# cychomatica/AudioPure

Hardware: AMD Instinct MI355X
Metric: purified 1s@16kHz utterances/sec at 5 reverse steps (higher is better)
Workload: dtype f32

## Files before the change

__graft_entry__.py:

```python
from __future__ import annotations

import glob
import os
import subprocess
import sys

ROOT = os.path.dirname(os.path.abspath(__file__))
if ROOT not in sys.path:
    sys.path.insert(0, ROOT)

CSRC = os.path.join(ROOT, "audiopure_amd", "csrc")
LIBDIR = os.path.join(ROOT, "audiopure_amd", "lib")
LIB = os.path.join(LIBDIR, "libaudiopure_hip.so")
TOOLS_LIB = os.path.join(ROOT, "tools", "lib", "libaudiopure_hip_tools.so")
NO_SLP_VECTORIZE = {"ap_resblock_f32w.hip", "ap_resblock_bwd.hip", "ap_resblock_bwd_bf16.hip", "ap_conv_w3.hip", "ap_conv_p1.hip",
                    "ap_resblock_bf16p.hip", "ap_resblock_bf16s.hip", "ap_resblock_bf16u.hip", "ap_resblock_bf16us.hip",
                    "ap_resblock_bf16.hip", "ap_resblock_bf16w.hip", "ap_resblock_f32w_parent.hip"}
TOOLS_CSRC = os.path.join(ROOT, "tools", "csrc")
TOOLS_ONLY_SOURCES = ["ap_resblock_bf16.hip", "ap_resblock_bf16w.hip", "ap_skipgemm_bf16w.hip", "ap_conv_p1.hip",
                      "ap_resblock_f32w_parent.hip"]
HIP_SOURCES = ["ap_kernels.hip", "ap_resblock_f32w.hip", "ap_resblock_bwd.hip", "ap_resblock_bwd_bf16.hip", "ap_resblock_bf16p.hip", "ap_resblock_bf16s.hip", "ap_resblock_bf16u.hip", "ap_resblock_bf16us.hip", "ap_skipgemm_bf16.hip", "ap_resblock_f32s.hip", "ap_resblock_f32s2.hip", "ap_capi.hip", "ap_frontend.hip", "ap_mel.hip", "ap_convnet.hip", "ap_conv_w3.hip", "ap_backward.hip", "ap_kws.hip", "ap_unet_bwd.hip", "ap_defense.hip", "ap_psy.hip", "ap_wgrad.hip", "ap_m5_train.hip", "ap_convnet_train.hip", "ap_unet_train.hip", "ap_optim.hip", "ap_loss.hip"]


def _newer(target: str, sources) -> bool:
    if not os.path.exists(target):
        return False
    t = os.path.getmtime(target)
    return all(os.path.getmtime(s) <= t for s in sources)


def hip_flags(src: str, tools: bool = False) -> list:
    return (["--offload-arch=gfx950", "-O3", "-std=c++17", "-fPIC", "-I", CSRC] + (["-DAP_TOOLS"] if tools else [])
            + (["-fno-slp-vectorize"] if os.path.basename(src) in NO_SLP_VECTORIZE else []))


def build_hip(force: bool = False, tools: bool = False) -> str:
    lib = TOOLS_LIB if tools else LIB
    variant = os.environ.get("AP_VARIANT_LIB")
    if variant:
        lib, force = os.path.abspath(variant), True
    os.makedirs(os.path.dirname(lib), exist_ok=True)
    srcs = [os.path.join(CSRC, f) for f in HIP_SOURCES if os.path.exists(os.path.join(CSRC, f))]
    if tools:
        srcs += [os.path.join(TOOLS_CSRC, f) for f in TOOLS_ONLY_SOURCES]
    deps = srcs + glob.glob(os.path.join(CSRC, "*.h")) + [os.path.join(ROOT, "include", "audiopure.h")]
    if not force and _newer(lib, deps):
        return lib
    hipcc = os.environ.get("HIPCC", "/opt/rocm/bin/hipcc")
    objs = []
    procs = []
    for s in srcs:
        o = os.path.join(os.path.dirname(lib), os.path.basename(s) + (".tools.o" if tools else ".var.o" if variant else ".o"))
        objs.append(o)
        cmd = ([hipcc] + hip_flags(s, tools) + (os.environ.get("AP_VARIANT_FLAGS", "").split() if variant else []) + ["-c", s, "-o", o])
        procs.append((cmd, subprocess.Popen(cmd, stdout=subprocess.PIPE, stderr=subprocess.STDOUT)))
    for cmd, p in procs:
        out, _ = p.communicate()
        if p.returncode != 0:
            raise RuntimeError("hipcc failed: " + " ".join(cmd) + "\n" + out.decode(errors="replace"))
    cmd = [hipcc, "--offload-arch=gfx950", "-shared", "-fPIC", "-o", lib] + objs
    subprocess.run(cmd, check=True)
    for o in objs:
        os.remove(o)
    return lib


def build_oracle() -> None:
    mk = os.path.join(ROOT, "oracle", "Makefile")
    if os.path.exists(mk):
        subprocess.run(["make", "-s", "-C", os.path.join(ROOT, "oracle")], check=True)


def build() -> None:
    have_hipcc = os.path.exists(os.environ.get("HIPCC", "/opt/rocm/bin/hipcc"))
    build_hip(force=have_hipcc and os.environ.get("AP_BUILD_REUSE") != "1")
    build_oracle()
    import audiopure_amd
    from audiopure_amd import _native
    _native.lib()


def smoke() -> None:
    import numpy as np
    import torch

    from audiopure_amd import synth
    from audiopure_amd.diffusion_models.diffwave_ddpm import DiffWave
    from audiopure_amd.diffusion_models.DiffWave_Unconditional.WaveNet import WaveNet_Speech_Commands
    from audiopure_amd.diffusion_models.DiffWave_Unconditional.util import calc_diffusion_hyperparams
    from audiopure_amd.audio_models.M5.M5Net import M5
    from audiopure_amd.acoustic_system import AcousticSystem
    from oracle import diffwave_oracle as O

    assert torch.cuda.is_available(), "smoke() needs a GPU"
    dev = torch.device("cuda:0")
    cfg = synth.mini_wavenet_config(64, 12, 12)
    sd = synth.wavenet_state_dict(cfg, 0)
    net = WaveNet_Speech_Commands(**cfg)
    net.load_state_dict({k: torch.from_numpy(v) for k, v in sd.items()})
    net = net.to(dev)
    dh = calc_diffusion_hyperparams(**synth.DIFFUSION_CONFIG)
    B, L, n = 2, 16000, 2
    x0 = torch.from_numpy(synth.waveforms(B, L, seed=11))
    z = [torch.from_numpy(synth.noise(d, B, L, seed=11)) for d in range(n)]
    dw = DiffWave(model=net, diffusion_hyperparams=dh, reverse_timestep=n)
    dw.set_noise_source(list(t.to(dev) for t in z))
    m5sd = synth.m5_state_dict(10)
    m5 = M5(n_input=1, n_output=10)
    m5.load_state_dict({k: torch.from_numpy(np.asarray(v)) for k, v in m5sd.items()})
    m5 = m5.to(dev).eval()
    system = AcousticSystem(classifier=m5, transform=None, defender=dw, defense_type="wave")
    logp = system(x0.to(dev), True).cpu()
    x_ref, lp_ref = O.purify_and_classify(O.fold_state_dict(sd), cfg, O.diffusion_hyperparams(**synth.DIFFUSION_CONFIG),
                                          m5sd, x0, n, z)
    err = (logp - lp_ref).abs().max().item()
    assert err < 1e-3, f"smoke: log-prob mismatch {err}"
    print(f"smoke OK: max |dlogp| = {err:.2e}")


if __name__ == "__main__":
    if "--tools" in sys.argv:
        print("tools build OK:", build_hip(force=True, tools=True))
    else:
        build()
        print("build OK:", LIB)
```

audiopure_amd/csrc/ap_kernels.hip:

```cpp
#include "ap_common.h"

namespace ap {

__global__ void rownorm_kernel(const float *__restrict__ v, float *__restrict__ norm, int O, int IK) {
  int row = blockIdx.x * (blockDim.x >> 6) + (threadIdx.x >> 6);
  int lane = threadIdx.x & 63;
  if (row >= O) return;
  const float *p = v + (size_t)row * IK;
  float s = 0.f;
  for (int i = lane; i < IK; i += 64) s = __builtin_fmaf(p[i], p[i], s);
  for (int o = 32; o > 0; o >>= 1) s += __shfl_xor(s, o);
  if (lane == 0) norm[row] = sqrtf(s);
}

__global__ void fold_kernel(const float *__restrict__ g, const float *__restrict__ v,
                            const float *__restrict__ norm, float *__restrict__ out, int O, int IK) {
  size_t idx = (size_t)blockIdx.x * blockDim.x + threadIdx.x;
  if (idx >= (size_t)O * IK) return;
  int o = idx / IK;
  out[idx] = v[idx] * (g[o] / norm[o]);
}

__global__ void pack_w1_kernel(const float *__restrict__ w1f, float *__restrict__ out, int C) {
  const int NW = C / 64, NG = C * 3 / 8;
  size_t idx = (size_t)blockIdx.x * blockDim.x + threadIdx.x;
  size_t total = (size_t)NW * NG * 4 * 64 * 4;
  if (idx >= total) return;
  int e = idx & 3;
  int lane = (idx >> 2) & 63;
  int rt = (idx >> 8) & 3;
  size_t rest = idx >> 10;
  int G = rest % NG;
  int w = rest / NG;
  int s = 4 * G + e, hh = lane >> 5, i = lane & 31;
  int kk = 2 * s + hh;
  int chunk = kk / (3 * KC), within = kk % (3 * KC);
  int tap = within / KC, cl = within % KC;
  int c = chunk * KC + cl;
  int o = (rt & 1) * C + 64 * w + 32 * (rt >> 1) + i;
  out[idx] = w1f[((size_t)o * C + c) * 3 + tap];
}

__global__ void pack_rows_kernel(const float *__restrict__ wf, float *__restrict__ out, int M, int K, int RT,
                                 int mode) {
  const int NG = K / 8;
  const int NWv = M / (32 * RT);
  size_t idx = (size_t)blockIdx.x * blockDim.x + threadIdx.x;
  size_t total = (size_t)NWv * NG * RT * 64 * 4;
  if (idx >= total) return;
  int e = idx & 3;
  int lane = (idx >> 2) & 63;
  size_t rest = idx >> 8;
  int rt = rest % RT;
  rest /= RT;
  int G = rest % NG;
  int w = rest / NG;
  int s = 4 * G + e, hh = lane >> 5, i = lane & 31;
  int kk = 2 * s + hh;
  int o = 32 * RT * w + 32 * rt + i;
  if (mode == 1) o = (rt >> 1) * (M / 2) + 64 * w + 32 * (rt & 1) + i;
  out[idx] = wf[(size_t)o * K + kk];
}

__global__ void copy_kernel(const float *__restrict__ in, float *__restrict__ out, size_t n) {
  size_t idx = (size_t)blockIdx.x * blockDim.x + threadIdx.x;
  if (idx < n) out[idx] = in[idx];
}

static int fold_one(const float *g, const float *v, float *norms, float *out, int O, int IK, hipStream_t st) {
  rownorm_kernel<<<(O + 3) / 4, 256, 0, st>>>(v, norms, O, IK);
  size_t n = (size_t)O * IK;
  fold_kernel<<<(unsigned)((n + 255) / 256), 256, 0, st>>>(g, v, norms, out, O, IK);
  return 0;
}

static void copy_to(const float *in, float *out, size_t n, hipStream_t st) {
  copy_kernel<<<(unsigned)((n + 255) / 256), 256, 0, st>>>(in, out, n);
}

int launch_fold_and_pack(ap_ctx *ctx, const float *blob, hipStream_t st) {
  const ap_config &c = ctx->cfg;
  const int C = ctx->C, S = ctx->S, NL = ctx->NL;
  BlobLayout bl = blob_layout(c);
  fold_one(blob + bl.init_g, blob + bl.init_v, ctx->norms, ctx->w0, C, 1, st);
  copy_to(blob + bl.init_b, ctx->b0, C, st);
  copy_to(blob + bl.fc1_w, ctx->fc1_w, (size_t)c.embed_dim_mid * c.embed_dim_in, st);
  copy_to(blob + bl.fc1_b, ctx->fc1_b, c.embed_dim_mid, st);
  copy_to(blob + bl.fc2_w, ctx->fc2_w, (size_t)c.embed_dim_out * c.embed_dim_mid, st);
  copy_to(blob + bl.fc2_b, ctx->fc2_b, c.embed_dim_out, st);
  for (int n = 0; n < NL; n++) {
    const float *b = blob + bl.blk0 + (size_t)n * bl.blk_stride;
    copy_to(b + bl.fct_w, ctx->fct_w + (size_t)n * C * c.embed_dim_out, (size_t)C * c.embed_dim_out, st);
    copy_to(b + bl.fct_b, ctx->fct_b + (size_t)n * C, C, st);
    float *w1f = ctx->w1f + (size_t)n * 2 * C * C * 3;
    float *w2f = ctx->w2f + (size_t)n * (C + S) * C;
    fold_one(b + bl.dil_g, b + bl.dil_v, ctx->norms, w1f, 2 * C, C * 3, st);
    fold_one(b + bl.res_g, b + bl.res_v, ctx->norms, w2f, C, C, st);
    fold_one(b + bl.skip_g, b + bl.skip_v, ctx->norms, w2f + (size_t)C * C, S, C, st);
    copy_to(b + bl.dil_b, ctx->b1 + (size_t)n * 2 * C, 2 * C, st);
    copy_to(b + bl.res_b, ctx->b2 + (size_t)n * (C + S), C, st);
    copy_to(b + bl.skip_b, ctx->b2 + (size_t)n * (C + S) + C, S, st);
    size_t n1 = (size_t)2 * C * C * 3, n2 = (size_t)(C + S) * C;
    pack_w1_kernel<<<(unsigned)((n1 + 255) / 256), 256, 0, st>>>(w1f, ctx->w1p + (size_t)n * n1, C);
    pack_rows_kernel<<<(unsigned)((n2 + 255) / 256), 256, 0, st>>>(w2f, ctx->w2p + (size_t)n * n2, C + S, C, 4, 1);
  }
  fold_one(blob + bl.f1_g, blob + bl.f1_v, ctx->norms, ctx->wf1f, S, S, st);
  copy_to(blob + bl.f1_b, ctx->bf1, S, st);
  copy_to(blob + bl.f2_w, ctx->wf2, S, st);
  copy_to(blob + bl.f2_b, ctx->bf2, 1, st);
  size_t nf = (size_t)S * S;
  pack_rows_kernel<<<(unsigned)((nf + 255) / 256), 256, 0, st>>>(ctx->wf1f, ctx->wf1p, S, S, 2, 0);
  AP_HIP(hipGetLastError());
  return 0;
}

__device__ __forceinline__ float swish_acc(float x) { return x / (1.0f + expf(-x)); }

__global__ __launch_bounds__(512) void embed_mlp_kernel(const float *__restrict__ freq, const float *__restrict__ w1,
                                                        const float *__restrict__ b1, const float *__restrict__ w2,
                                                        const float *__restrict__ b2, float step, int Ein, int Emid,
                                                        int Eout, float *__restrict__ emb_out) {
  extern __shared__ float sm[];
  float *e0 = sm, *e1 = sm + Ein;
  const int lane = threadIdx.x & 63, wave = threadIdx.x >> 6;
  int half = Ein / 2;
  for (int i = threadIdx.x; i < half; i += blockDim.x) {
    float a = step * freq[i];
    e0[i] = sinf(a);
    e0[half + i] = cosf(a);
  }
  __syncthreads();
  for (int o0 = wave; o0 < Emid; o0 += 8 * 16) {
    float s[16];
#pragma unroll
    for (int i = 0; i < 16; i++) s[i] = 0.f;
    for (int kk = 0; kk < Ein; kk += 64) {
      const int k = min(kk + lane, Ein - 1);
      const float ev = kk + lane < Ein ? e0[k] : 0.f;
#pragma unroll
      for (int i = 0; i < 16; i++) s[i] = __builtin_fmaf(w1[(size_t)min(o0 + 8 * i, Emid - 1) * Ein + k], ev, s[i]);
    }
    for (int m = 32; m > 0; m >>= 1) {
#pragma unroll
      for (int i = 0; i < 16; i++) s[i] += __shfl_xor(s[i], m);
    }
    float mine = 0.f;
#pragma unroll
    for (int i = 0; i < 16; i++) mine = lane == i ? s[i] : mine;
    const int o = o0 + 8 * lane;
    if (lane < 16 && o < Emid) e1[o] = swish_acc(mine + b1[o]);
  }
  __syncthreads();
  const int o2 = min((int)blockIdx.x * 8 + wave, Eout - 1);
  float s = 0.f;
  for (int kk = 0; kk < Emid; kk += 512) {
    float wv[8];
#pragma unroll
    for (int i = 0; i < 8; i++) wv[i] = w2[(size_t)o2 * Emid + min(kk + 64 * i + lane, Emid - 1)];
#pragma unroll
    for (int i = 0; i < 8; i++) s = kk + 64 * i + lane < Emid ? __builtin_fmaf(wv[i], e1[kk + 64 * i + lane], s) : s;
  }
  for (int m = 32; m > 0; m >>= 1) s += __shfl_xor(s, m);
  if (lane == 0 && (int)blockIdx.x * 8 + wave < Eout) emb_out[o2] = swish_acc(s + b2[o2]);
}

__global__ void fct_kernel(const float *__restrict__ w, const float *__restrict__ b, const float *__restrict__ emb,
                           float *__restrict__ out, int rows, int E) {
  int row = blockIdx.x * (blockDim.x >> 6) + (threadIdx.x >> 6);
  int lane = threadIdx.x & 63;
  if (row >= rows) return;
  const float *p = w + (size_t)row * E;
  float s = 0.f;
  for (int i0 = 0; i0 < E; i0 += 512) {
    float wv[8], ev[8];
#pragma unroll
    for (int u = 0; u < 8; u++) {
      const int i = min(i0 + 64 * u + lane, E - 1);
      wv[u] = p[i];
      ev[u] = emb[i];
    }
#pragma unroll
    for (int u = 0; u < 8; u++) s = i0 + 64 * u + lane < E ? __builtin_fmaf(wv[u], ev[u], s) : s;
  }
  for (int o = 32; o > 0; o >>= 1) s += __shfl_xor(s, o);
  if (lane == 0) out[row] = s + b[row];
}

int launch_embed(ap_ctx *ctx, float step, float *part_t, hipStream_t st) {
  const ap_config &c = ctx->cfg;
  float *emb = part_t + (size_t)ctx->NL * ctx->C;
  size_t sm = (size_t)(c.embed_dim_in + c.embed_dim_mid) * sizeof(float);
  embed_mlp_kernel<<<(unsigned)((c.embed_dim_out + 7) / 8), 512, sm, st>>>(ctx->emb_freq, ctx->fc1_w, ctx->fc1_b, ctx->fc2_w, ctx->fc2_b, step,
                                       c.embed_dim_in, c.embed_dim_mid, c.embed_dim_out, emb);
  int rows = ctx->NL * ctx->C;
  fct_kernel<<<(rows + 3) / 4, 256, 0, st>>>(ctx->fct_w, ctx->fct_b, emb, part_t, rows, c.embed_dim_out);
  AP_HIP(hipGetLastError());
  return 0;
}

__global__ void init_conv_kernel(const float *__restrict__ x, const float *__restrict__ w0,
                                 const float *__restrict__ b0, float *__restrict__ h, int C, int L) {
  int b = blockIdx.z, c = blockIdx.y;
  int t = blockIdx.x * blockDim.x + threadIdx.x;
  if (t >= L) return;
  float v = __builtin_fmaf(w0[c], x[(size_t)b * L + t], b0[c]);
  h[((size_t)b * C + c) * L + t] = fmaxf(v, 0.f);
}

int launch_init_conv(ap_ctx *ctx, const float *x, float *h, int B, int L, hipStream_t st) {
  dim3 grid((L + 255) / 256, ctx->C, B);
  init_conv_kernel<<<grid, 256, 0, st>>>(x, ctx->w0, ctx->b0, h, ctx->C, L);
  AP_HIP(hipGetLastError());
  return 0;
}

template <int C, int TTK>
struct RBGeom {
  static constexpr int NWM = C / 64;
  static constexpr int NWN = TTK / 64;
  static constexpr int NW = NWM * NWN;
  static constexpr int NT = NW * 64;
  static constexpr int ROWS = 3 * KC;
  static constexpr int NCHUNK = C / KC;
  static constexpr int GPC = ROWS / 8;
  static constexpr int NG1 = NCHUNK * GPC;
  static constexpr int NG2 = C / 8;
  static constexpr int EPT = ROWS * TTK / NT;
  static constexpr int RPI = NT / TTK;
  static constexpr int NPT = KC / RPI;
  static constexpr int XBUF = ROWS * TTK;
  static constexpr int LDS_FLOATS = (2 * XBUF > C * TTK) ? 2 * XBUF : C * TTK;
};

template <int C, int TTK, bool SAVE = false>
__global__ __launch_bounds__(C / 64 * TTK, 2) void resblock_f32_kernel(
    const float *__restrict__ hin, const float *__restrict__ pt, float *__restrict__ hout, float *__restrict__ skip,
    const float *__restrict__ w1p, const float *__restrict__ b1, const float *__restrict__ w2p,
    const float *__restrict__ b2, int L, int d, int accumulate, int ntiles, float *__restrict__ aout AP_ABLATE_PARAM) {
  AP_ABLATE_DECL
  using G = RBGeom<C, TTK>;
  constexpr int TT = TTK;
  constexpr int NT = G::NT;
  __shared__ float lds[G::LDS_FLOATS];

  const int tid = threadIdx.x;
  const int lane = tid & 63;
  const int wave = __builtin_amdgcn_readfirstlane(tid >> 6);
  const int mw = wave / G::NWN, nw = wave % G::NWN;
  const int j = lane & 31, hh = lane >> 5;
  int b_, tile_;
  ap_tile_of_block(blockIdx.x, gridDim.x, ntiles, d, TT, b_, tile_);
  const int b = __builtin_amdgcn_readfirstlane(b_);
  const int t0 = __builtin_amdgcn_readfirstlane(tile_ * TT);
  const float *hin_b;
  {
    const uint64_t hb = (uint64_t)(hin + (size_t)b * C * L);
    const uint32_t lo = __builtin_amdgcn_readfirstlane((uint32_t)hb);
    const uint32_t hi = __builtin_amdgcn_readfirstlane((uint32_t)(hb >> 32));
    hin_b = (const float *)(((uint64_t)hi << 32) | lo);
  }

  f32x16 acc[4][2];
#pragma unroll
  for (int rt = 0; rt < 4; rt++) {
    const int obase = (rt & 1) * C + 64 * mw + 32 * (rt >> 1);
#pragma unroll
    for (int q = 0; q < 4; q++) {
      const float4 bv = *reinterpret_cast<const float4 *>(b1 + obase + 8 * q + 4 * hh);
#pragma unroll
      for (int ct = 0; ct < 2; ct++) {
        acc[rt][ct][4 * q + 0] = bv.x;
        acc[rt][ct][4 * q + 1] = bv.y;
        acc[rt][ct][4 * q + 2] = bv.z;
        acc[rt][ct][4 * q + 3] = bv.w;
      }
    }
  }

  constexpr int RPI = G::RPI, NPT = G::NPT;
  const int rsel = tid / TT;
  unsigned voff[3];
  bool tok[3];
#pragma unroll
  for (int tap = 0; tap < 3; tap++) {
    const int tp = t0 + (tid & (TT - 1)) + (tap - 1) * d;
    tok[tap] = (tp >= 0) && (tp < L);
    voff[tap] = ((unsigned)min(max(tp, 0), L - 1) + (unsigned)rsel * (unsigned)L) * 4u;
  }
  const __amdgpu_buffer_rsrc_t hrs =
      __builtin_amdgcn_make_buffer_rsrc((void *)hin_b, 0, (int)((unsigned)C * (unsigned)L * 4u), 0x00020000);
  float xr[G::EPT];
  float ptv[NPT];
  auto issue_loads = [&](int ch) {
#pragma unroll
    for (int q = 0; q < NPT; q++) ptv[q] = pt[ch * KC + q * RPI + rsel];
#pragma unroll
    for (int i = 0; i < G::EPT; i++) {
      const int rowc = i * RPI;
      const int tap = rowc / KC, clc = rowc % KC;
      const int soff = (ch * KC + clc) * L * 4;
      xr[i] = __builtin_bit_cast(float, __builtin_amdgcn_raw_buffer_load_b32(hrs, voff[tap], soff, 0));
    }
  };
  auto store_chunk = [&](float *dst) {
#pragma unroll
    for (int i = 0; i < G::EPT; i++) {
      const int rowc = i * RPI;
      const int tap = rowc / KC, clc = rowc % KC;
      const float u = xr[i] + ptv[clc / RPI];
      dst[i * NT + tid] = tok[tap] ? u : 0.f;
    }
  };

  issue_loads(0);
  store_chunk(lds);
  __syncthreads();

  auto load_a = [&](f32x4(&a)[4], const f32x4 *base, int Gi) {
#pragma unroll
    for (int rt = 0; rt < 4; rt++) a[rt] = base[(size_t)((ablate & 4) ? 0 : Gi) * 256 + rt * 64];
  };
  auto mma4 = [&](const f32x4(&a)[4], const float *xb) {
    float bv[4][2];
#pragma unroll
    for (int e = 0; e < 4; e++)
#pragma unroll
      for (int ct = 0; ct < 2; ct++) bv[e][ct] = xb[e * 2 * TT + 32 * ct];
#pragma unroll
    for (int e = 0; e < 4; e++)
#pragma unroll
      for (int rt = 0; rt < 4; rt++)
#pragma unroll
        for (int ct = 0; ct < 2; ct++)
          acc[rt][ct] = __builtin_amdgcn_mfma_f32_32x32x2f32(a[rt][e], bv[e][ct], acc[rt][ct], 0, 0, 0);
  };

  const int colbase = 64 * nw + j;
  const f32x4 *ap = reinterpret_cast<const f32x4 *>(w1p) + (size_t)mw * G::NG1 * 4 * 64 + lane;
  f32x4 a0[4], a1[4];
  load_a(a0, ap, 0);
  {
    static_assert(G::GPC % 2 == 0 && G::NG1 % 2 == 0, "pair-unrolled loop");
    int ch = 0, g = 0;
#pragma unroll 1
    for (int Gi = 0; Gi < G::NG1; Gi += 2) {
      load_a(a1, ap, Gi + 1);
      if (g == 0 && ch + 1 < G::NCHUNK && !(ablate & 8)) issue_loads(ch + 1);
      __builtin_amdgcn_sched_barrier(0);
      const float *xb = lds + (ch & 1) * G::XBUF + (g * 8 + hh) * TT + colbase;
      mma4(a0, xb);
      __builtin_amdgcn_sched_barrier(0);
      load_a(a0, ap, (Gi + 2 < G::NG1) ? Gi + 2 : Gi);
      __builtin_amdgcn_sched_barrier(0);
      mma4(a1, xb + 8 * TT);
      __builtin_amdgcn_sched_barrier(0);
      g += 2;
      if (g == G::GPC) {
        if (ch + 1 < G::NCHUNK) store_chunk(lds + ((ch + 1) & 1) * G::XBUF);
        __syncthreads();
        g = 0;
        ch++;
      }
    }
  }

#pragma unroll
  for (int p = 0; p < 2; p++)
#pragma unroll
    for (int ct = 0; ct < 2; ct++) {
#pragma unroll
      for (int r = 0; r < 16; r++) {
        const int c = 64 * mw + 32 * p + rowoff(r, hh);
        if constexpr (SAVE) {
          const int t = t0 + 32 * ct + colbase;
          if (t < L) {
            float *ab = aout + ((size_t)b * 2 * C + c) * L + t;
            ab[0] = acc[2 * p][ct][r];
            ab[(size_t)C * L] = acc[2 * p + 1][ct][r];
          }
        }
        lds[c * TT + 32 * ct + colbase] =
            (ablate & 2) ? acc[2 * p][ct][r] : gate(acc[2 * p][ct][r], acc[2 * p + 1][ct][r]);
      }
      __builtin_amdgcn_sched_barrier(0);
    }

  {
    const float *b2l = b2, *ptl = pt;
    asm volatile("" : "+s"(b2l), "+s"(ptl));
#pragma unroll
    for (int rt = 0; rt < 4; rt++) {
      const int cb = 64 * mw + 32 * (rt & 1);
#pragma unroll
      for (int q = 0; q < 4; q++) {
        const int c = cb + 8 * q + 4 * hh;
        float4 bv = *reinterpret_cast<const float4 *>(b2l + (rt < 2 ? 0 : C) + c);
        if (rt < 2) {
          const float4 pv = *reinterpret_cast<const float4 *>(ptl + c);
          bv.x += pv.x; bv.y += pv.y; bv.z += pv.z; bv.w += pv.w;
        }
#pragma unroll
        for (int ct = 0; ct < 2; ct++) {
          acc[rt][ct][4 * q + 0] = bv.x;
          acc[rt][ct][4 * q + 1] = bv.y;
          acc[rt][ct][4 * q + 2] = bv.z;
          acc[rt][ct][4 * q + 3] = bv.w;
        }
      }
    }
  }
  const f32x4 *ap2 = reinterpret_cast<const f32x4 *>(w2p) + (size_t)mw * G::NG2 * 4 * 64 + lane;
  load_a(a0, ap2, 0);
  load_a(a1, ap2, 1);
  __syncthreads();

  float hres[2][2][16];
  unsigned evoff[2][2];
#pragma unroll
  for (int rt = 0; rt < 2; rt++)
#pragma unroll
    for (int ct = 0; ct < 2; ct++) {
      const int t = min(t0 + 32 * ct + colbase, L - 1);
      evoff[rt][ct] = ((unsigned)(64 * mw + 32 * rt + 4 * hh) * (unsigned)L + (unsigned)t) * 4u;
    }
  if (!(ablate & 1)) {
#pragma unroll
    for (int rt = 0; rt < 2; rt++)
#pragma unroll
      for (int ct = 0; ct < 2; ct++)
#pragma unroll
        for (int r = 0; r < 16; r++)
          hres[rt][ct][r] = __builtin_bit_cast(
              float, __builtin_amdgcn_raw_buffer_load_b32(hrs, evoff[rt][ct], rowoff(r, 0) * L * 4, 2));
  }

  {
    static_assert(G::NG2 % 2 == 0, "pair-unrolled loop");
#pragma unroll 1
    for (int Gi = 0; Gi < G::NG2; Gi += 2) {
      const float *gb = lds + (Gi * 8 + hh) * TT + colbase;
      mma4(a0, gb);
      __builtin_amdgcn_sched_barrier(0);
      load_a(a0, ap2, (Gi + 2 < G::NG2) ? Gi + 2 : Gi);
      __builtin_amdgcn_sched_barrier(0);
      mma4(a1, gb + 8 * TT);
      __builtin_amdgcn_sched_barrier(0);
      load_a(a1, ap2, (Gi + 3 < G::NG2) ? Gi + 3 : Gi + 1);
      __builtin_amdgcn_sched_barrier(0);
    }
  }

  if (ablate & 1) return;
  const float RS = 0.707106781186547524f;
  float *ho = hout + (size_t)b * C * L;
  float *sk = skip + (size_t)b * C * L;
#pragma unroll
  for (int rt = 0; rt < 4; rt++) {
#pragma unroll
    for (int ct = 0; ct < 2; ct++) {
      const int t = t0 + 32 * ct + colbase;
      const unsigned rbase = (unsigned)(64 * mw + 32 * (rt & 1) + 4 * hh) * (unsigned)L + (unsigned)t;
      if (t < L) {
        if (rt < 2) {
#pragma unroll
          for (int r = 0; r < 16; r++)
            __builtin_nontemporal_store((hres[rt][ct][r] + acc[rt][ct][r]) * RS, &ho[rbase + (unsigned)rowoff(r, 0) * (unsigned)L]);
        } else if (accumulate) {
#pragma unroll
          for (int r = 0; r < 16; r++)
            unsafeAtomicAdd(&sk[rbase + (unsigned)rowoff(r, 0) * (unsigned)L], acc[rt][ct][r]);
        } else {
#pragma unroll
          for (int r = 0; r < 16; r++) __builtin_nontemporal_store(acc[rt][ct][r], &sk[rbase + (unsigned)rowoff(r, 0) * (unsigned)L]);
        }
      }
    }
  }
}

AP_TOOLS_VAR g_tile = 64;
AP_TOOLS_VAR g_force_direct = 0;
AP_TOOLS_VAR g_no_bf16s = 0;
AP_TOOLS_VAR g_force_f32 = 0;
#ifdef AP_TOOLS
static int g_ablate = 0;
#endif

int launch_resblock(ap_ctx *ctx, int layer, const float *hin, const float *pt, float *hout, float *skip,
                    int accumulate, int B, int L, hipStream_t st, float *aout, void *gout, void *fout) {
  if (aout && ctx->cfg.precision != AP_PREC_F32) {
    set_error("ap_resblock_fwd_save: AP_PREC_F32 only (the other modes recompute the pre-gate activations)");
    return -22;
  }
  if (ctx->cfg.precision == AP_PREC_BF16_STORE) {
    set_error("AP_PREC_BF16_STORE: the residual stream is a bf16 image in this mode (ap_init_conv_u / ap_resblock_fwd_u), not an fp32 tensor; "
              "the fp32-tensor block serves AP_PREC_F32, AP_PREC_F32_SPLIT and AP_PREC_BF16");
    return -22;
  }
  if (gout && (ctx->cfg.precision != AP_PREC_BF16 || g_force_f32)) {
    set_error("deferred-skip form: AP_PREC_BF16 only");
    return -22;
  }
  if (ctx->cfg.precision != AP_PREC_F32 && !g_force_f32) {
    ProfileSpan span;
    if (int e = span.begin(ctx, 0, st)) return e;
    int rc = ctx->cfg.precision == AP_PREC_BF16
                 ? (gout && !fout && g_no_bf16s != 1 && (g_no_bf16s == 2 || resblock_bf16s_serves(ctx, B, L))
                        ? launch_resblock_bf16s(ctx, layer, hin, pt, hout, gout, B, L, st)
                        : launch_resblock_bf16(ctx, layer, hin, pt, hout, skip, accumulate, B, L, st, gout, fout))
                 : launch_resblock_split(ctx, layer, hin, pt, hout, skip, accumulate, B, L, st);
    if (int e = span.end()) return e;
    return rc;
  }
  const int C = ctx->C, S = ctx->S;
  const int d = 1 << (layer % ctx->cfg.dilation_cycle);
  if (!g_force_direct && resblock_f32w_serves(ctx, B, L)) {
    ProfileSpan span;
    if (int e = span.begin(ctx, 0, st)) return e;
    const int rcw = launch_resblock_f32w(ctx, layer, hin, pt, hout, skip, accumulate, B, L, st, aout);
    if (int e = span.end()) return e;
    return rcw;
  }
  if (!hout) {
    set_error("resblock: the direct-form block needs an h' buffer");
    return -22;
  }
  const float *w1p = ctx->w1p + (size_t)layer * 2 * C * C * 3;
  const float *w2p = ctx->w2p + (size_t)layer * (C + S) * C;
  const float *b1 = ctx->b1 + (size_t)layer * 2 * C;
  const float *b2 = ctx->b2 + (size_t)layer * (C + S);
  ProfileSpan span;
  if (int e = span.begin(ctx, 0, st)) return e;
#define AP_RB(CC, TK)                                                                                              \
  resblock_f32_kernel<CC, TK><<<(unsigned)B * ((L + TK - 1) / TK), CC / 64 * TK, 0, st>>>(                         \
      hin, pt, hout, skip, w1p, b1, w2p, b2, L, d, accumulate, (L + TK - 1) / TK, nullptr AP_ABLATE_ARG(g_ablate))
#define AP_RB_SAVE(CC, TK)                                                                                         \
  resblock_f32_kernel<CC, TK, true><<<(unsigned)B * ((L + TK - 1) / TK), CC / 64 * TK, 0, st>>>(                   \
      hin, pt, hout, skip, w1p, b1, w2p, b2, L, d, accumulate, (L + TK - 1) / TK, aout AP_ABLATE_ARG(g_ablate))
  const int tk = g_tile;
  if (aout) {
    if (C == 256 && tk == 64) AP_RB_SAVE(256, 64);
    else if (C == 256) AP_RB_SAVE(256, 128);
    else if (C == 64) AP_RB_SAVE(64, 64);
    else {
      set_error("resblock (save): unsupported res_channels %d (need 64 or 256)", C);
      return -22;
    }
  } else
  if (C == 64 && tk == 64) AP_RB(64, 64);
  else if (C == 64) AP_RB(64, 128);
  else if (C == 128 && tk == 64) AP_RB(128, 64);
  else if (C == 128) AP_RB(128, 128);
  else if (C == 256 && tk == 64) AP_RB(256, 64);
  else if (C == 256) AP_RB(256, 128);
  else {
    set_error("resblock: unsupported res_channels %d (need 64, 128 or 256)", C);
    return -22;
  }
#undef AP_RB
#undef AP_RB_SAVE
  if (int e = span.end()) return e;
  AP_HIP(hipGetLastError());
  return 0;
}

__device__ __forceinline__ void philox4x32_10(uint32_t c0, uint32_t c1, uint32_t c2, uint32_t c3, uint32_t k0,
                                              uint32_t k1, uint32_t (&out)[4]) {
#pragma unroll
  for (int i = 0; i < 10; i++) {
    uint32_t hi0 = __umulhi(0xD2511F53u, c0), lo0 = 0xD2511F53u * c0;
    uint32_t hi1 = __umulhi(0xCD9E8D57u, c2), lo1 = 0xCD9E8D57u * c2;
    uint32_t n0 = hi1 ^ c1 ^ k0, n1 = lo1, n2 = hi0 ^ c3 ^ k1, n3 = lo0;
    c0 = n0; c1 = n1; c2 = n2; c3 = n3;
    k0 += 0x9E3779B9u;
    k1 += 0xBB67AE85u;
  }
  out[0] = c0; out[1] = c1; out[2] = c2; out[3] = c3;
}

__device__ __forceinline__ void philox_normal4(uint64_t seed, uint32_t draw, uint64_t utt, uint32_t quad,
                                               float (&z)[4]) {
  uint32_t r[4];
  philox4x32_10(quad, draw, (uint32_t)utt, (uint32_t)(utt >> 32), (uint32_t)seed, (uint32_t)(seed >> 32), r);
  const float TWO_PI = 6.283185307179586f;
#pragma unroll
  for (int p = 0; p < 2; p++) {
    float u1 = ((float)(r[2 * p] >> 9) + 0.5f) * 1.1920928955078125e-07f;
    float u2 = (float)(r[2 * p + 1] >> 8) * 5.9604644775390625e-08f;
    float rad = sqrtf(-2.0f * logf(u1));
    float sn, cs;
    sincosf(TWO_PI * u2, &sn, &cs);
    z[2 * p] = rad * cs;
    z[2 * p + 1] = rad * sn;
  }
}

__device__ __forceinline__ float philox_normal1(uint64_t seed, uint32_t draw, uint64_t utt, int t) {
  float z[4];
  philox_normal4(seed, draw, utt, (uint32_t)t >> 2, z);
  return z[t & 3];
}

__global__ void affine_noise_kernel(const float *__restrict__ x, float *__restrict__ out, float ca, float cs,
                                    const float *__restrict__ z, uint64_t seed, uint32_t draw, uint64_t utt_offset,
                                    int L) {
  const int b = blockIdx.y;
  const int q = blockIdx.x * blockDim.x + threadIdx.x;
  const int t = q * 4;
  if (t >= L) return;
  float zz[4];
  if (z == nullptr) {
    if (cs != 0.f) philox_normal4(seed, draw, utt_offset + b, (uint32_t)q, zz);
    else zz[0] = zz[1] = zz[2] = zz[3] = 0.f;
  }
#pragma unroll
  for (int i = 0; i < 4; i++) {
    if (t + i < L) {
      const size_t off = (size_t)b * L + t + i;
      float zv = z ? z[off] : zz[i];
      float xv = x ? x[off] : 0.f;
      out[off] = ca * xv + cs * zv;
    }
  }
}

int launch_affine_noise(const float *x, float *out, float ca, float cs, const float *z, uint64_t seed,
                        uint32_t draw, uint64_t utt_offset, int B, int L, hipStream_t st) {
  int quads = (L + 3) / 4;
  dim3 grid((quads + 255) / 256, B);
  affine_noise_kernel<<<grid, 256, 0, st>>>(x, out, ca, cs, z, seed, draw, utt_offset, L);
  AP_HIP(hipGetLastError());
  return 0;
}

template <int S, int FT>
__global__ __launch_bounds__(S / 64 * 64, FT == 64 ? 2 : 1) void final_f32_kernel(
    const float *__restrict__ skip, const float *__restrict__ x, float *__restrict__ eps_out, float *__restrict__ out,
    const float *__restrict__ wf1p, const float *__restrict__ bf1, const float *__restrict__ wf2,
    const float *__restrict__ bf2, float scale, float ca, float cb, float cs, const float *__restrict__ z,
    uint64_t seed, uint32_t draw, uint64_t utt_offset, int L, int ntiles) {
  constexpr int NW = S / 64, NT = NW * 64, NG = S / 8;
  constexpr int TT = FT, NCT = FT / 32;
  __shared__ float lds[S * TT];
  const int tid = threadIdx.x, lane = tid & 63;
  const int wave = __builtin_amdgcn_readfirstlane(tid >> 6);
  const int j = lane & 31, hh = lane >> 5;
  const int b = blockIdx.x / ntiles;
  const int t0 = (blockIdx.x % ntiles) * TT;
  const float *sk = skip + (size_t)b * S * L;

  for (int e = tid; e < S * TT; e += NT) {
    const int row = e / TT, col = e % TT;
    const int t = t0 + col;
    lds[e] = (t < L) ? sk[(size_t)row * L + t] * scale : 0.f;
  }
  f32x16 acc[2][NCT];
#pragma unroll
  for (int rt = 0; rt < 2; rt++)
#pragma unroll
    for (int r = 0; r < 16; r++) {
      float bv = bf1[64 * wave + 32 * rt + rowoff(r, hh)];
#pragma unroll
      for (int ct = 0; ct < NCT; ct++) acc[rt][ct][r] = bv;
    }
  __syncthreads();

  const f32x4 *ap = reinterpret_cast<const f32x4 *>(wf1p) + (size_t)wave * NG * 2 * 64 + lane;
  f32x4 a_cur[2], a_nxt[2];
  a_cur[0] = ap[0];
  a_cur[1] = ap[64];
#pragma unroll 2
  for (int Gi = 0; Gi < NG; Gi++) {
    if (Gi + 1 < NG) {
      a_nxt[0] = ap[(size_t)(Gi + 1) * 128];
      a_nxt[1] = ap[(size_t)(Gi + 1) * 128 + 64];
    }
#pragma unroll
    for (int e = 0; e < 4; e++) {
      const int s = Gi * 4 + e;
      float bv[NCT];
#pragma unroll
      for (int ct = 0; ct < NCT; ct++) bv[ct] = lds[(2 * s + hh) * TT + 32 * ct + j];
#pragma unroll
      for (int rt = 0; rt < 2; rt++)
#pragma unroll
        for (int ct = 0; ct < NCT; ct++)
          acc[rt][ct] = __builtin_amdgcn_mfma_f32_32x32x2f32(a_cur[rt][e], bv[ct], acc[rt][ct], 0, 0, 0);
    }
    a_cur[0] = a_nxt[0];
    a_cur[1] = a_nxt[1];
  }
  float part[NCT];
#pragma unroll
  for (int ct = 0; ct < NCT; ct++) part[ct] = 0.f;
#pragma unroll
  for (int rt = 0; rt < 2; rt++)
#pragma unroll
    for (int r = 0; r < 16; r++) {
      const float w = wf2[64 * wave + 32 * rt + rowoff(r, hh)];
#pragma unroll
      for (int ct = 0; ct < NCT; ct++) part[ct] = __builtin_fmaf(fmaxf(acc[rt][ct][r], 0.f), w, part[ct]);
    }
#pragma unroll
  for (int ct = 0; ct < NCT; ct++) part[ct] += __shfl_xor(part[ct], 32);
  __syncthreads();
  if (hh == 0) {
#pragma unroll
    for (int ct = 0; ct < NCT; ct++) lds[wave * TT + 32 * ct + j] = part[ct];
  }
  __syncthreads();
  for (int col = tid; col < TT; col += NT) {
    const int t = t0 + col;
    if (t < L) {
      float e = bf2[0];
#pragma unroll
      for (int w = 0; w < NW; w++) e += lds[w * TT + col];
      const size_t off = (size_t)b * L + t;
      if (eps_out) eps_out[off] = e;
      if (out) {
        float v = ca * x[off] + cb * e;
        if (cs != 0.f) {
          float zv = z ? z[off] : philox_normal1(seed, draw, utt_offset + b, t);
          v += cs * zv;
        }
        out[off] = v;
      }
    }
  }
}

typedef __bf16 fb16x8 __attribute__((ext_vector_type(8)));
__global__ __launch_bounds__(256, 2) void final_bf16_kernel(
    const float *__restrict__ skip, const float *__restrict__ x, float *__restrict__ eps_out, float *__restrict__ out,
    const fb16x8 *__restrict__ wfp, const float *__restrict__ bf1, const float *__restrict__ wf2,
    const float *__restrict__ bf2, float scale, float ca, float cb, float cs, const float *__restrict__ z, uint64_t seed,
    uint32_t draw, uint64_t utt_offset, int L, int ntiles) {
  constexpr int S = 256, FT = 64, NW = 4, RB = S * 2 + 16, NKS = S / 16;
  __shared__ __attribute__((aligned(16))) unsigned char img[FT * RB];
  __shared__ float red[NW * FT];
  const int tid = threadIdx.x, lane = tid & 63;
  const int wave = __builtin_amdgcn_readfirstlane(tid >> 6);
  const int j = lane & 31, hh = lane >> 5;
  const int b = blockIdx.x / ntiles;
  const int t0 = (blockIdx.x % ntiles) * FT;
  const float *sk = skip + (size_t)b * S * L;
#pragma unroll
  for (int r = 0; r < 2; r++) {
    const int item = tid + 256 * r, cq = item & 15, oct = item >> 4;
    const int t = t0 + 4 * cq;
    float v[8][4];
#pragma unroll
    for (int e = 0; e < 8; e++) {
      const float *row = sk + (size_t)(oct * 8 + e) * L;
      if ((L & 3) == 0) {
        const float4 q = t < L ? *reinterpret_cast<const float4 *>(row + t) : make_float4(0.f, 0.f, 0.f, 0.f);
        v[e][0] = q.x; v[e][1] = q.y; v[e][2] = q.z; v[e][3] = q.w;
      } else {
#pragma unroll
        for (int i = 0; i < 4; i++) v[e][i] = t + i < L ? row[t + i] : 0.f;
      }
    }
#pragma unroll
    for (int i = 0; i < 4; i++) {
      fb16x8 pk;
#pragma unroll
      for (int e = 0; e < 8; e++) pk[e] = (__bf16)(v[e][i] * scale);
      *reinterpret_cast<fb16x8 *>(img + (4 * cq + i) * RB + oct * 16) = pk;
    }
  }
  f32x16 acc[2][2];
#pragma unroll
  for (int rt = 0; rt < 2; rt++)
#pragma unroll
    for (int r = 0; r < 16; r++) {
      const float bv = bf1[64 * wave + 32 * rt + rowoff(r, hh)];
      acc[rt][0][r] = bv;
      acc[rt][1][r] = bv;
    }
  __syncthreads();
  const fb16x8 *ap = wfp + (size_t)(wave * 2) * NKS * 64 + lane;
  fb16x8 a0[2], a1[2], a2[2];
  a0[0] = ap[0]; a0[1] = ap[NKS * 64];
  a1[0] = ap[64]; a1[1] = ap[NKS * 64 + 64];
  const unsigned char *bp = img + j * RB + 16 * hh;
  auto kstep = [&](const fb16x8(&a)[2], int ks) {
    fb16x8 bv[2];
#pragma unroll
    for (int ct = 0; ct < 2; ct++) bv[ct] = *reinterpret_cast<const fb16x8 *>(bp + (32 * ct) * RB + ks * 32);
#pragma unroll
    for (int rt = 0; rt < 2; rt++)
#pragma unroll
      for (int ct = 0; ct < 2; ct++) acc[rt][ct] = __builtin_amdgcn_mfma_f32_32x32x16_bf16(a[rt], bv[ct], acc[rt][ct], 0, 0, 0);
  };
  auto fetch = [&](fb16x8(&a)[2], int ks) {
    const int k2 = ks < NKS ? ks : NKS - 1;
    a[0] = ap[k2 * 64];
    a[1] = ap[NKS * 64 + k2 * 64];
  };
#pragma unroll 1
  for (int ks = 0; ks < NKS; ks += 3) {
    fetch(a2, ks + 2);
    kstep(a0, ks);
    if (ks + 1 < NKS) {
      fetch(a0, ks + 3);
      kstep(a1, ks + 1);
    }
    if (ks + 2 < NKS) {
      fetch(a1, ks + 4);
      kstep(a2, ks + 2);
    }
  }
  float part[2] = {0.f, 0.f};
#pragma unroll
  for (int rt = 0; rt < 2; rt++)
#pragma unroll
    for (int r = 0; r < 16; r++) {
      const float w = wf2[64 * wave + 32 * rt + rowoff(r, hh)];
#pragma unroll
      for (int ct = 0; ct < 2; ct++) part[ct] = __builtin_fmaf(fmaxf(acc[rt][ct][r], 0.f), w, part[ct]);
    }
#pragma unroll
  for (int ct = 0; ct < 2; ct++) part[ct] += __shfl_xor(part[ct], 32);
  if (hh == 0) {
#pragma unroll
    for (int ct = 0; ct < 2; ct++) red[wave * FT + 32 * ct + j] = part[ct];
  }
  __syncthreads();
  if (tid < FT) {
    const int t = t0 + tid;
    if (t < L) {
      float e = bf2[0];
#pragma unroll
      for (int w = 0; w < NW; w++) e += red[w * FT + tid];
      const size_t off = (size_t)b * L + t;
      if (eps_out) eps_out[off] = e;
      if (out) {
        float v = ca * x[off] + cb * e;
        if (cs != 0.f) {
          const float zv = z ? z[off] : philox_normal1(seed, draw, utt_offset + b, t);
          v += cs * zv;
        }
        out[off] = v;
      }
    }
  }
}

int launch_final_affine_bf16(ap_ctx *ctx, const float *skip, const float *x, float *eps_out, float *out, float ca, float cb,
                             float cs, const float *z, uint64_t seed, uint32_t draw, uint64_t utt_offset, int B, int L,
                             hipStream_t st) {
  if (ctx->S != 256 || !ctx->wf1p_bf) return 1;
  const int ntiles = (L + 63) / 64;
  const float scale = (float)sqrt(1.0 / (double)ctx->NL);
  final_bf16_kernel<<<(unsigned)B * ntiles, 256, 0, st>>>(skip, x, eps_out, out, (const fb16x8 *)ctx->wf1p_bf, ctx->bf1, ctx->wf2,
                                                          ctx->bf2, scale, ca, cb, cs, z, seed, draw, utt_offset, L, ntiles);
  AP_HIP(hipGetLastError());
  return 0;
}

int launch_final_affine(ap_ctx *ctx, const float *skip, const float *x, float *eps_out, float *out, float ca,
                        float cb, float cs, const float *z, uint64_t seed, uint32_t draw, uint64_t utt_offset,
                        int B, int L, hipStream_t st) {
  if (ctx->cfg.precision == AP_PREC_BF16 || ctx->cfg.precision == AP_PREC_BF16_STORE) {
    const int rc = launch_final_affine_bf16(ctx, skip, x, eps_out, out, ca, cb, cs, z, seed, draw, utt_offset, B, L, st);
    if (rc != 1) return rc;
  }
  const int S = ctx->S;
  const int ft = (S == 256) ? 64 : TT;
  const int ntiles = (L + ft - 1) / ft;
  const float scale = (float)sqrt(1.0 / (double)ctx->NL);
  unsigned grid = (unsigned)B * ntiles;
#define AP_FINAL(SS, FTV)                                                                                         \
  final_f32_kernel<SS, FTV><<<grid, SS, 0, st>>>(skip, x, eps_out, out, ctx->wf1p, ctx->bf1, ctx->wf2, ctx->bf2,   \
                                                 scale, ca, cb, cs, z, seed, draw, utt_offset, L, ntiles)
  switch (S) {
    case 64: AP_FINAL(64, 128); break;
    case 128: AP_FINAL(128, 128); break;
    case 256: AP_FINAL(256, 64); break;
    default:
      set_error("final: unsupported skip_channels %d", S);
      return -22;
  }
#undef AP_FINAL
  AP_HIP(hipGetLastError());
  return 0;
}

__global__ void nes_perturb_kernel(const float *__restrict__ x, float *__restrict__ out, float sigma, uint64_t seed,
                                   uint32_t draw, int S, int lead, int L) {
  const int a = blockIdx.z, s = blockIdx.y;
  const int q = blockIdx.x * blockDim.x + threadIdx.x, t = 4 * q;
  if (t >= L) return;
  const int half = S / 2, sp = s - lead;
  float zz[4] = {0.f, 0.f, 0.f, 0.f};
  float sgn = 0.f;
  if (sp >= 0) {
    const int p = sp < half ? sp : sp - half;
    sgn = sp < half ? sigma : -sigma;
    philox_normal4(seed, draw, (uint64_t)a * half + p, (uint32_t)q, zz);
  }
  const float *xa = x + (size_t)a * L;
  float *o = out + ((size_t)a * (S + lead) + s) * L;
#pragma unroll
  for (int i = 0; i < 4; i++)
    if (t + i < L) o[t + i] = __builtin_fmaf(sgn, zz[i], xa[t + i]);
}

__global__ void nes_grad_kernel(const float *__restrict__ loss, float *__restrict__ grad, uint64_t seed, uint32_t draw,
                                int S, int L, int accumulate) {
  const int a = blockIdx.y;
  const int q = blockIdx.x * blockDim.x + threadIdx.x, t = 4 * q;
  if (t >= L) return;
  const int half = S / 2;
  float acc[4] = {0.f, 0.f, 0.f, 0.f};
  for (int p = 0; p < half; p++) {
    float zz[4];
    philox_normal4(seed, draw, (uint64_t)a * half + p, (uint32_t)q, zz);
    const float w = loss[(size_t)a * S + p] - loss[(size_t)a * S + half + p];
#pragma unroll
    for (int i = 0; i < 4; i++) acc[i] = __builtin_fmaf(w, zz[i], acc[i]);
  }
  float *g = grad + (size_t)a * L;
#pragma unroll
  for (int i = 0; i < 4; i++)
    if (t + i < L) g[t + i] = (accumulate ? g[t + i] : 0.f) + acc[i] / (float)S;
}

__global__ void philox_fill_kernel(float *__restrict__ out, uint64_t seed, uint32_t draw, uint64_t utt_offset,
                                   int L) {
  const int b = blockIdx.y;
  const int t = blockIdx.x * blockDim.x + threadIdx.x;
  if (t < L) out[(size_t)b * L + t] = philox_normal1(seed, draw, utt_offset + b, t);
}

}

#ifdef AP_TOOLS
extern "C" int ap_debug_tile(int tile) {
  if (tile != 64 && tile != 128) return -22;
  ap::g_tile = tile;
  return 0;
}

extern "C" int ap_debug_force_f32(int on) {
  ap::g_force_f32 = on;
  return 0;
}

extern "C" int ap_debug_no_bf16s(int on) {
  ap::g_no_bf16s = on;
  return 0;
}

namespace ap { extern int g_ablate_bf16; extern int g_dbg_bf16; extern unsigned long long *g_trace_bf16; }
extern "C" int ap_debug_bf16_dbg(int bits) {
  ap::g_dbg_bf16 = bits;
  return 0;
}

extern "C" int ap_debug_trace(void *buf) {
  ap::g_trace_bf16 = (unsigned long long *)buf;
  return 0;
}

extern "C" int ap_debug_ablate(int mask) {
  ap::g_ablate = mask;
  ap::g_ablate_bf16 = mask;
  return 0;
}
#endif

extern "C" int ap_nes_perturb(const float *x, float *out, float sigma, uint64_t seed, uint32_t draw, int A, int S,
                              int lead, int L, void *stream) {
  if (!x || !out || A < 1 || S < 2 || (S & 1) || L < 1 || lead < 0 || lead > 1) { ap::set_error("ap_nes_perturb: bad argument"); return -22; }
  dim3 grid((unsigned)(((L + 3) / 4 + 255) / 256), (unsigned)(S + lead), (unsigned)A);
  ap::nes_perturb_kernel<<<grid, 256, 0, (hipStream_t)stream>>>(x, out, sigma, seed, draw, S, lead, L);
  AP_HIP(hipGetLastError());
  return 0;
}

extern "C" int ap_nes_grad(const float *loss, float *grad, uint64_t seed, uint32_t draw, int A, int S, int L,
                           int accumulate, void *stream) {
  if (!loss || !grad || A < 1 || S < 2 || (S & 1) || L < 1) { ap::set_error("ap_nes_grad: bad argument"); return -22; }
  dim3 grid((unsigned)(((L + 3) / 4 + 255) / 256), (unsigned)A);
  ap::nes_grad_kernel<<<grid, 256, 0, (hipStream_t)stream>>>(loss, grad, seed, draw, S, L, accumulate);
  AP_HIP(hipGetLastError());
  return 0;
}

extern "C" int ap_philox_normal(float *out, uint64_t seed, uint32_t draw, uint64_t utt_offset, int B, int L,
                                void *stream) {
  dim3 grid((L + 255) / 256, B);
  ap::philox_fill_kernel<<<grid, 256, 0, (hipStream_t)stream>>>(out, seed, draw, utt_offset, L);
  AP_HIP(hipGetLastError());
  return 0;
}
```

Baseline: 60.55.

## Add vectorized f32 final-projection kernel for 256 skip channels

Adds a specialized f32 kernel for the final skip-to-eps projection when skip channels are 256. It loads the skip tile with 16-byte vector reads into registers, transposes it into padded shared memory, and software-pipelines the weight and B-operand loads ahead of the f32 MFMA loop. It also prefetches x and z before the matrix work so those loads overlap. The fast path applies only when L is a multiple of 4 and skip is 16-byte aligned, and it adds register pressure.

```diff
diff --git a/__graft_entry__.py b/__graft_entry__.py
--- a/__graft_entry__.py
+++ b/__graft_entry__.py
@@ -18,7 +18,7 @@
                     "ap_resblock_bf16.hip", "ap_resblock_bf16w.hip", "ap_resblock_f32w_parent.hip"}
 TOOLS_CSRC = os.path.join(ROOT, "tools", "csrc")
 TOOLS_ONLY_SOURCES = ["ap_resblock_bf16.hip", "ap_resblock_bf16w.hip", "ap_skipgemm_bf16w.hip", "ap_conv_p1.hip",
-                      "ap_resblock_f32w_parent.hip"]
+                      "ap_resblock_f32w_parent.hip", "ap_final_f32_parent.hip"]
 HIP_SOURCES = ["ap_kernels.hip", "ap_resblock_f32w.hip", "ap_resblock_bwd.hip", "ap_resblock_bwd_bf16.hip", "ap_resblock_bf16p.hip", "ap_resblock_bf16s.hip", "ap_resblock_bf16u.hip", "ap_resblock_bf16us.hip", "ap_skipgemm_bf16.hip", "ap_resblock_f32s.hip", "ap_resblock_f32s2.hip", "ap_capi.hip", "ap_frontend.hip", "ap_mel.hip", "ap_convnet.hip", "ap_conv_w3.hip", "ap_backward.hip", "ap_kws.hip", "ap_unet_bwd.hip", "ap_defense.hip", "ap_psy.hip", "ap_wgrad.hip", "ap_m5_train.hip", "ap_convnet_train.hip", "ap_unet_train.hip", "ap_optim.hip", "ap_loss.hip"]
 
 
diff --git a/audiopure_amd/csrc/ap_kernels.hip b/audiopure_amd/csrc/ap_kernels.hip
--- a/audiopure_amd/csrc/ap_kernels.hip
+++ b/audiopure_amd/csrc/ap_kernels.hip
@@ -729,6 +729,116 @@
   }
 }
 
+__global__ __launch_bounds__(256, 2) void final_f32q_kernel(
+    const float *__restrict__ skip, const float *__restrict__ x, float *__restrict__ eps_out, float *__restrict__ out,
+    const float *__restrict__ wf1p, const float *__restrict__ bf1, const float *__restrict__ wf2,
+    const float *__restrict__ bf2, float scale, float ca, float cb, float cs, const float *__restrict__ z,
+    uint64_t seed, uint32_t draw, uint64_t utt_offset, int L, int ntiles) {
+  constexpr int S = 256, FT = 64, NW = 4, NG = S / 8, P = S + 4;
+  __shared__ __attribute__((aligned(16))) float img[FT * P];
+  __shared__ float red[NW * FT];
+  __shared__ __attribute__((aligned(16))) float cst[2 * S];
+  const int tid = threadIdx.x, lane = tid & 63;
+  const int wave = __builtin_amdgcn_readfirstlane(tid >> 6);
+  const int j = lane & 31, hh = lane >> 5;
+  const int b = blockIdx.x / ntiles;
+  const int t0 = (blockIdx.x % ntiles) * FT;
+  cst[tid] = bf1[tid];
+  cst[S + tid] = wf2[tid];
+  const int cq = tid & 15, gq = tid >> 4;
+  const bool in = t0 + 4 * cq < L;
+  const float *sk = skip + ((size_t)b * S + 8 * (gq >> 1) + (gq & 1)) * L + t0 + (in ? 4 * cq : 0);
+  f32x4 xq[4][4];
+#pragma unroll
+  for (int r = 0; r < 4; r++)
+#pragma unroll
+    for (int e = 0; e < 4; e++) xq[r][e] = *reinterpret_cast<const f32x4 *>(sk + (size_t)(64 * r + 2 * e) * L);
+  const f32x4 *ap = reinterpret_cast<const f32x4 *>(wf1p) + (size_t)wave * NG * 2 * 64 + lane;
+  f32x4 a[4][2], bb[2][2];
+#pragma unroll
+  for (int g = 0; g < 2; g++)
+#pragma unroll
+    for (int rt = 0; rt < 2; rt++) a[g][rt] = ap[g * 128 + rt * 64];
+  const int tcol = t0 + lane;
+  const size_t off = (size_t)b * L + tcol;
+  float xu = 0.f, zu = 0.f;
+  if (wave == 0 && tcol < L && out) {
+    xu = x[off];
+    if (cs != 0.f && z) zu = z[off];
+  }
+#pragma unroll
+  for (int r = 0; r < 4; r++)
+#pragma unroll
+    for (int i = 0; i < 4; i++) {
+      f32x4 o;
+#pragma unroll
+      for (int e = 0; e < 4; e++) o[e] = in ? xq[r][e][i] * scale : 0.f;
+      *reinterpret_cast<f32x4 *>(img + (4 * cq + i) * P + 4 * (gq + 16 * r)) = o;
+    }
+  __syncthreads();
+  f32x16 acc[2][2];
+#pragma unroll
+  for (int rt = 0; rt < 2; rt++)
+#pragma unroll
+    for (int r = 0; r < 16; r++) {
+      const float bv = cst[64 * wave + 32 * rt + rowoff(r, hh)];
+      acc[rt][0][r] = bv;
+      acc[rt][1][r] = bv;
+    }
+  const float *bp = img + j * P + 4 * hh;
+#pragma unroll
+  for (int ct = 0; ct < 2; ct++) bb[0][ct] = *reinterpret_cast<const f32x4 *>(bp + 32 * ct * P);
+#pragma unroll
+  for (int G = 0; G < NG; G++) {
+    if (G + 2 < NG) {
+#pragma unroll
+      for (int rt = 0; rt < 2; rt++) a[(G + 2) & 3][rt] = ap[(G + 2) * 128 + rt * 64];
+    }
+    if (G + 1 < NG) {
+#pragma unroll
+      for (int ct = 0; ct < 2; ct++) bb[(G + 1) & 1][ct] = *reinterpret_cast<const f32x4 *>(bp + 32 * ct * P + 8 * (G + 1));
+    }
+#pragma unroll
+    for (int e = 0; e < 4; e++)
+#pragma unroll
+      for (int rt = 0; rt < 2; rt++)
+#pragma unroll
+        for (int ct = 0; ct < 2; ct++)
+          acc[rt][ct] = __builtin_amdgcn_mfma_f32_32x32x2f32(a[G & 3][rt][e], bb[G & 1][ct][e], acc[rt][ct], 0, 0, 0);
+    __builtin_amdgcn_sched_barrier(0);
+  }
+  float part[2] = {0.f, 0.f};
+#pragma unroll
+  for (int rt = 0; rt < 2; rt++)
+#pragma unroll
+    for (int r = 0; r < 16; r++) {
+      const float w = cst[S + 64 * wave + 32 * rt + rowoff(r, hh)];
+#pragma unroll
+      for (int ct = 0; ct < 2; ct++) part[ct] = __builtin_fmaf(fmaxf(acc[rt][ct][r], 0.f), w, part[ct]);
+    }
+#pragma unroll
+  for (int ct = 0; ct < 2; ct++) part[ct] += __shfl_xor(part[ct], 32);
+  if (hh == 0) {
+#pragma unroll
+    for (int ct = 0; ct < 2; ct++) red[wave * FT + 32 * ct + j] = part[ct];
+  }
+  __syncthreads();
+  if (wave == 0 && tcol < L) {
+    float e = bf2[0];
+#pragma unroll
+    for (int w = 0; w < NW; w++) e += red[w * FT + lane];
+    if (eps_out) eps_out[off] = e;
+    if (out) {
+      float v = ca * xu + cb * e;
+      if (cs != 0.f) {
+        float zv = z ? zu : philox_normal1(seed, draw, utt_offset + b, tcol);
+        v += cs * zv;
+      }
+      out[off] = v;
+    }
+  }
+}
+
 typedef __bf16 fb16x8 __attribute__((ext_vector_type(8)));
 __global__ __launch_bounds__(256, 2) void final_bf16_kernel(
     const float *__restrict__ skip, const float *__restrict__ x, float *__restrict__ eps_out, float *__restrict__ out,
@@ -866,6 +976,14 @@
     if (rc != 1) return rc;
   }
   const int S = ctx->S;
+  if (S == 256 && L % 4 == 0 && ((uintptr_t)skip & 15) == 0) {
+    const int ntiles = (L + 63) / 64;
+    const float scale = (float)sqrt(1.0 / (double)ctx->NL);
+    final_f32q_kernel<<<(unsigned)B * ntiles, 256, 0, st>>>(skip, x, eps_out, out, ctx->wf1p, ctx->bf1, ctx->wf2, ctx->bf2, scale, ca, cb, cs,
+                                                           z, seed, draw, utt_offset, L, ntiles);
+    AP_HIP(hipGetLastError());
+    return 0;
+  }
   const int ft = (S == 256) ? 64 : TT;
   const int ntiles = (L + ft - 1) / ft;
   const float scale = (float)sqrt(1.0 / (double)ctx->NL);
```

Result: no change. 60.77, median of 6 (+0.4%).
